# ctlab/metacherchant

Hardware: AMD Instinct MI355X
Metric: k-mers/s processed (count+BFS) at k=31 (higher is better)
Workload: dtype int64

## Files before the change

metacherchant_amd/csrc/count_pipeline.h:

```cpp
#pragma once
#include <utility>
#include "kmer_device.h"

namespace mc {

constexpr int PT_THREADS = 1024;
constexpr int PT_ITEMS = 8;
constexpr int PT_TILE = PT_THREADS * PT_ITEMS;
constexpr int PT_MAX_BUCKETS = 512;
constexpr int PT_MAX_BUCKETS_KEYS = 1024;
constexpr int PT_MAX_LEAVES2 = 1024;
constexpr int PT_MAX_BUCKETS1_SK = 2048;
constexpr int SK_LEAVES_LG = 21;
constexpr int P3_THREADS = 512;
constexpr uint32_t REGION_SLOTS = 1u << MC_REGION_LG;
constexpr uint32_t CURSOR1_STRIDE = 32;
constexpr int PT_SEGMENTS = 256;

__host__ __device__ __forceinline__ uint32_t mulhi32(uint32_t bin, uint32_t n) { return (uint32_t)(((uint64_t)bin * n) >> 32); }

struct ScatterLds {
    uint64_t key[PT_TILE];
    uint32_t hint[PT_TILE];
    uint32_t rel[PT_TILE];
// ... 437 lines not shown

#ifndef MC_P1W_MIN_WAVES
#define MC_P1W_MIN_WAVES 4
#endif
#ifndef MC_P1W_PREFETCH_WORDS
#define MC_P1W_PREFETCH_WORDS 1
#endif
#ifndef MC_P1W_COMPACT
#define MC_P1W_COMPACT 1
#endif
#ifndef MC_P1W_THREADS
#define MC_P1W_THREADS 1024
#endif
constexpr int P1W_THREADS = MC_P1W_THREADS;
constexpr int P1W_WAVES = P1W_THREADS / 64;
constexpr uint32_t P1W_TILE = 62 * PT_ITEMS;
constexpr int P1W_SEGMENTS = 1024;
static_assert(PT_MAX_LEAVES2 <= PT_THREADS && PT_MAX_BUCKETS_KEYS <= PT_THREADS, "one thread per leaf cursor");
static_assert(P1W_SEGMENTS <= PT_THREADS && P1W_SEGMENTS >= PT_SEGMENTS, "k_sk2_scatter scans one segment count per thread");

__device__ __forceinline__ uint32_t wave_incl_sum(uint32_t v)
{
    v += (uint32_t)__builtin_amdgcn_update_dpp(0, (int)v, 0x111, 0xF, 0xF, true);
    v += (uint32_t)__builtin_amdgcn_update_dpp(0, (int)v, 0x112, 0xF, 0xF, true);
    v += (uint32_t)__builtin_amdgcn_update_dpp(0, (int)v, 0x114, 0xF, 0xF, true);
    v += (uint32_t)__builtin_amdgcn_update_dpp(0, (int)v, 0x118, 0xF, 0xF, true);
    v += (uint32_t)__builtin_amdgcn_update_dpp(0, (int)v, 0x142, 0xA, 0xF, false);
    v += (uint32_t)__builtin_amdgcn_update_dpp(0, (int)v, 0x143, 0xC, 0xF, false);
    return v;
}

// ... 15 lines not shown
__device__ __forceinline__ uint32_t sk_start_bits(uint32_t lane, uint32_t valid, uint32_t brk)
{
    static_assert(N <= 16 && N <= (int)MAXW && (MAXW & (MAXW - 1)) == 0 && MAXW <= 32, "one deep start a lane at most");
    const unsigned long long holders = __ballot(brk != 0);
    const unsigned long long below = holders & ((1ull << lane) - 1ull);
    const uint32_t P = below ? 63u - (uint32_t)__builtin_clzll(below) : 0u;
    const uint32_t bp = (uint32_t)__shfl((int)brk, (int)P);
    const uint32_t cur = P * N + (31u - (uint32_t)__builtin_clz(bp | 1u));
    const uint32_t low = (brk & (0u - brk)) - 1u;
    const uint32_t deep = (1u << ((cur - lane * N) & (MAXW - 1u))) & low;
    return valid & (brk | deep);
}

__device__ __forceinline__ uint32_t p1w_wave(uint32_t tid) { return (uint32_t)__builtin_amdgcn_readfirstlane((int)(tid >> 6)); }

struct alignas(16) Sk1wLds {
    uint32_t wcur[PT_MAX_BUCKETS1_SK];
    uint32_t starts[P1W_WAVES][24];
    uint32_t brk[P1W_WAVES][20];
#if MC_P1W_COMPACT
    uint64_t wst[P1W_WAVES][24];
    uint32_t hst[P1W_WAVES][64 * PT_ITEMS];
    uint16_t squeue[P1W_WAVES][64 * PT_ITEMS];
#endif
};

__device__ __forceinline__ uint32_t wave_from_next(uint32_t x)
{
    return (uint32_t)__builtin_amdgcn_update_dpp(0, (int)x, 0x130, 0xF, 0xF, true);
}
__device__ __forceinline__ uint32_t wave_from_prev(uint32_t x, uint32_t first)
{
    return (uint32_t)__builtin_amdgcn_update_dpp((int)first, (int)x, 0x138, 0xF, 0xF, false);
}

__device__ __forceinline__ uint64_t p1w_bits(uint64_t W0, uint64_t W1, uint64_t W2, uint32_t q)
{
    const bool up = q >= 32;
    const uint64_t a = up ? W1 : W0, b = up ? W2 : W1;
    const uint32_t sh = 2 * (q & 31);
    return (a << sh) | ((b >> 1) >> (63 - sh));
}

constexpr uint32_t SKC_REL_BITS = 22;
constexpr uint32_t SKB_MAX_CELLS = 16384;
template <bool ON> struct Sk1wFine { uint32_t h[ON ? SKB_MAX_CELLS : 1]; uint32_t win[ON ? PT_MAX_BUCKETS : 1]; };
struct SkBinned { uint32_t sub, fine; uint32_t *fine_rows; unsigned long long *owner_windows; };
template <bool OWNERS, bool COMPACT = false, bool BINNED = false>
__global__ void __launch_bounds__(P1W_THREADS, MC_P1W_MIN_WAVES) k_sk1w_extract(
    const uint64_t *__restrict__ words, const uint64_t *__restrict__ offsets, uint64_t n_reads, uint64_t base_lo,
    uint64_t n_bases, uint64_t n_tiles, const uint32_t *__restrict__ first_read, int k, uint32_t np1, uint32_t *seg_counts,
    uint64_t cap, uint4 *out_recs, uint32_t *out_ptrs, SkSpill sp, uint64_t ptr_base, uint32_t chunk_tiles = 0, uint32_t m2 = 0,
    SkBinned bn = SkBinned{1, 1, nullptr, nullptr})
{
    static_assert(!(OWNERS && COMPACT), "the compact form is for the single-GPU pipeline");
    static_assert(!BINNED || OWNERS, "fine buckets are the owners' business");
    __shared__ Sk1wLds L;
    __shared__ Sk1wFine<BINNED> F;
    const uint32_t tid = threadIdx.x, lane = tid & 63u, wv = p1w_wave(tid);
    for (uint32_t i = tid; i < PT_MAX_BUCKETS1_SK; i += P1W_THREADS) L.wcur[i] = 0;
    if (BINNED) {
        for (uint32_t i = tid; i < np1 * bn.fine; i += P1W_THREADS) F.h[i] = 0;
        for (uint32_t i = tid; i < np1; i += P1W_THREADS) F.win[i] = 0;
    }
    auto bucket_of = [&](uint32_t hsel, uint32_t bin, uint32_t n_win) -> uint32_t {
        if (BINNED) {
            const uint32_t o = sk_owner(hsel, np1);
            atomicAdd(&F.h[o * bn.fine + mulhi32(bin, bn.fine)], 1u);
            atomicAdd(&F.win[o], n_win);
            return o * bn.sub + mulhi32(bin, bn.sub);
        }
        return OWNERS ? sk_owner(hsel, np1) : mulhi32(bin, np1);
    };
    uint32_t *starts = L.starts[wv];
    uint32_t *brkw = L.brk[wv];
    uint8_t *brkb = reinterpret_cast<uint8_t *>(brkw);
#if MC_P1W_COMPACT
    uint64_t *wst = L.wst[wv];
    uint32_t *hst = L.hst[wv];
    uint16_t *squeue = L.squeue[wv];
    if (lane < 24) wst[lane] = 0;
#endif
    if (lane < 20) brkw[lane] = lane == 0 ? 0u : 0xFFFFFFFFu;
    __syncthreads();
    const int w = k - SK_M + 1;
    const uint64_t last_word = (n_bases + 31) / 32;
    const uint64_t seg_base = (uint64_t)blockIdx.x * cap, bucket_stride = (uint64_t)gridDim.x * cap;
    const uint64_t wave_id = (uint64_t)blockIdx.x * P1W_WAVES + wv, n_waves = (uint64_t)gridDim.x * P1W_WAVES;

    uint64_t pfW0 = 0, pfW1 = 0, pfW2 = 0, pf_off = ~0ull;
    uint32_t pf_first = 0;
    auto load_words = [&](uint64_t tile) {
        const int64_t p0 = (int64_t)(tile * P1W_TILE) + (int64_t)lane * PT_ITEMS;
        const int64_t wi0 = (p0 - 7) >> 5;
        pfW0 = wi0 >= 0 ? words[min((uint64_t)wi0, last_word)] : 0ull;
        pfW1 = words[min((uint64_t)(wi0 + 1), last_word)];
        pfW2 = words[min((uint64_t)(wi0 + 2), last_word)];
    };
    auto prefetch = [&](uint64_t tile) {
        if (tile >= n_tiles) return;
        if (MC_P1W_PREFETCH_WORDS) load_words(tile);
        pf_first = first_read[tile];
        const uint64_t r = (uint64_t)pf_first + lane;
        pf_off = r < n_reads ? offsets[r] : ~0ull;
    };
    const uint64_t chunk_lo = base_lo / P1W_TILE + (uint64_t)blockIdx.x * chunk_tiles;
    const uint64_t tile_end = COMPACT ? min(n_tiles, chunk_lo + chunk_tiles) : n_tiles;
    const uint64_t tile0 = COMPACT ? chunk_lo + wv : base_lo / P1W_TILE + wave_id;
    const uint64_t tile_step = COMPACT ? (uint64_t)P1W_WAVES : n_waves;
    prefetch(tile0);
    for (uint64_t tile = tile0; tile < tile_end; tile += tile_step) {
        const uint64_t lo = tile * (uint64_t)P1W_TILE;
        const int64_t bm_lo = (int64_t)lo - 64;
        const uint64_t bm_hi = lo + 640;
        if (!MC_P1W_PREFETCH_WORDS) load_words(tile);
        const uint64_t W0 = pfW0, W1 = pfW1, W2 = pfW2;
        uint64_t s = pf_off;
        const uint32_t my_first = pf_first;
        prefetch(tile + tile_step);
        const uint64_t p0 = lo + (uint64_t)lane * PT_ITEMS;
        const uint32_t off0 = (uint32_t)((int64_t)p0 - 32 * (((int64_t)p0 - 7) >> 5));

        if (lane < 24) starts[lane] = 0;
        __builtin_amdgcn_fence(__ATOMIC_RELEASE, "wavefront");
        __builtin_amdgcn_wave_barrier();
        for (uint64_t r = (uint64_t)my_first + lane;; r += 64) {
            const bool in = r < n_reads && s < bm_hi;
            if (in) {
                const int64_t rel = (int64_t)s - bm_lo;
                if (rel >= 0) atomicOr(&starts[(uint32_t)rel >> 5], 1u << ((uint32_t)rel & 31));
            }
            if (__ballot(!in)) break;
            s = r + 64 < n_reads ? offsets[r + 64] : ~0ull;
        }
        __builtin_amdgcn_fence(__ATOMIC_RELEASE, "wavefront");
        __builtin_amdgcn_wave_barrier();
        uint32_t ws[4];
        {
            const uint32_t bit0 = lane * 8 + 56, wd = bit0 >> 5, sh = bit0 & 31;
            const uint32_t d0 = starts[wd], d1 = starts[wd + 1], d2 = starts[wd + 2], d3 = starts[wd + 3], d4 = starts[wd + 4];
            ws[0] = __builtin_amdgcn_alignbit(d1, d0, sh);
            ws[1] = __builtin_amdgcn_alignbit(d2, d1, sh);
            ws[2] = __builtin_amdgcn_alignbit(d3, d2, sh);
            ws[3] = __builtin_amdgcn_alignbit(d4, d3, sh);
        }

        uint32_t hh[24];
        {
            const uint64_t A = p1w_bits(W0, W1, W2, off0);
            uint32_t f = (uint32_t)(A >> (64 - 2 * SK_M)), r = sk_rc_mmer(f);
            hh[0] = sk_order(f < r ? f : r);
#pragma unroll
            for (int i = 1; i < 8; i++) {
                const uint32_t nb = (uint32_t)(A >> (62 - 2 * (i + SK_M - 1))) & 3u;
                f = ((f << 2) | nb) & SK_MMASK;
                r = (r >> 2) | ((3u - nb) << (2 * (SK_M - 1)));
                hh[i] = sk_order(f < r ? f : r);
            }
#pragma unroll
            for (int i = 0; i < 8; i++) hh[8 + i] = wave_from_next(hh[i]);
#pragma unroll
            for (int i = 0; i < 8; i++) hh[16 + i] = wave_from_next(hh[8 + i]);
        }
        uint32_t hmin[PT_ITEMS];
#define SK_CASE(W)                                                                             \
    case W: {                                                                                  \
        uint32_t core = hh[7];                                                                 \
        _Pragma("unroll") for (int i = 8; i < W; i++) core = min(core, hh[i]);                 \
        uint32_t suf = SK_NONE;                                                                \
        hmin[7] = core;                                                                        \
        _Pragma("unroll") for (int j = 6; j >= 0; j--) { suf = min(suf, hh[j]); hmin[j] = min(suf, core); } \
        uint32_t pre = SK_NONE;                                                                \
        _Pragma("unroll") for (int j = 1; j < PT_ITEMS; j++) { pre = min(pre, hh[W + j - 1]); hmin[j] = min(hmin[j], pre); } \
    } break;
        switch (w) {
            SK_CASE(9) SK_CASE(10) SK_CASE(11) SK_CASE(12) SK_CASE(13) SK_CASE(14) SK_CASE(15) SK_CASE(16)
        default:
            SK_CASE(17)
        }
#undef SK_CASE

        uint32_t valid_bits;
        {
            uint64_t S = ((((uint64_t)ws[1]) << 32) | ws[0]) >> 9;
            uint32_t width = 1;
            for (; 2 * width <= (uint32_t)k - 1; width *= 2) S |= S >> width;
            S |= S >> ((uint32_t)k - 1 - width);
            uint32_t edge = lane < 62 ? 0xFFu : 0u;
            if (lo < base_lo || lo + P1W_TILE + (uint64_t)k > n_bases + 1) {
                edge = 0;
                if (lane < 62 && p0 + (uint64_t)k <= n_bases) {
                    const uint64_t jmax = n_bases - (uint64_t)k - p0;
                    const uint32_t jm = jmax < 7 ? (uint32_t)jmax : 7u;
                    const uint32_t j0 = p0 >= base_lo ? 0u : (base_lo - p0 < 8 ? (uint32_t)(base_lo - p0) : 8u);
                    edge = ((2u << jm) - 1u) & ~((1u << j0) - 1u) & 0xFFu;
                }
            }
            valid_bits = ~(uint32_t)S & edge;
        }
        const uint32_t last = (valid_bits >> (PT_ITEMS - 1)) & 1u ? hmin[PT_ITEMS - 1] : SK_NONE;
        const uint32_t prev = wave_from_prev(last, SK_NONE);
        const uint32_t brk_bits = sk_break_bits<PT_ITEMS, false>(hmin, valid_bits, prev);
        brkb[2 + lane] = (uint8_t)brk_bits;
        __builtin_amdgcn_fence(__ATOMIC_RELEASE, "wavefront");
        __builtin_amdgcn_wave_barrier();
        const uint32_t start_bits = sk_start_bits<PT_ITEMS, SK_MAX_WINDOWS>(lane, valid_bits, brk_bits);

#if MC_P1W_COMPACT
        {
            const uint32_t cnt = (uint32_t)__builtin_popcount(start_bits);
            const uint32_t incl = wave_incl_sum(cnt);
            const uint32_t total = (uint32_t)__builtin_amdgcn_readlane((int)incl, 63);
            uint32_t at = incl - cnt;
            for (uint32_t todo = start_bits; todo; todo &= todo - 1) squeue[at++] = (uint16_t)(lane * PT_ITEMS + (uint32_t)__builtin_ctz(todo));
            const uint32_t r7 = (uint32_t)(((int64_t)lo - 7) & 31);
            const uint32_t idx0 = (r7 + lane * PT_ITEMS) >> 5;
            wst[idx0] = W0; wst[idx0 + 1] = W1; wst[idx0 + 2] = W2;
            *reinterpret_cast<uint4 *>(&hst[lane * PT_ITEMS]) = make_uint4(hmin[0], hmin[1], hmin[2], hmin[3]);
            *reinterpret_cast<uint4 *>(&hst[lane * PT_ITEMS + 4]) = make_uint4(hmin[4], hmin[5], hmin[6], hmin[7]);
            __builtin_amdgcn_fence(__ATOMIC_RELEASE, "wavefront");
            __builtin_amdgcn_wave_barrier();
            for (uint32_t i = lane; i < total; i += 64) {
                const uint32_t wi = squeue[i];
                const uint32_t b0 = 17u + wi;
                const uint32_t ahead = __builtin_amdgcn_alignbit(brkw[(b0 >> 5) + 1], brkw[b0 >> 5], b0 & 31u) & 0x7FFFu;
                const uint32_t n = ahead ? (uint32_t)__builtin_ctz(ahead) + 1u : SK_MAX_WINDOWS;
                const uint32_t len = n + (uint32_t)k - 1;
                const uint32_t q = wi + 7u + r7, wq = q >> 5, sh = 2u * (q & 31u);
                const uint64_t A = wst[wq], B = wst[wq + 1], C = wst[wq + 2];
                const uint64_t X0 = (A << sh) | ((B >> 1) >> (63u - sh)), X1 = (B << sh) | ((C >> 1) >> (63u - sh));
                uint64_t hi = X0 >> 4;
                uint32_t tail = (uint32_t)(((X0 & 0xFull) << 28) | (X1 >> 36));
                if (len <= 30) { hi &= ~0ull << (60 - 2 * len); tail = 0; }
                else tail &= len >= 46 ? ~0u : ~0u << (2 * (46 - len));
// ... 29 lines not shown
        }
        for (uint32_t todo = start_bits; todo; todo &= todo - 1) {
            const uint32_t j = (uint32_t)__builtin_ctz(todo);
            const uint32_t ahead = (uint32_t)(bw >> (17 + j)) & 0x7FFFu;
            const uint32_t n = ahead ? (uint32_t)__builtin_ctz(ahead) + 1u : SK_MAX_WINDOWS;
            const uint32_t len = n + (uint32_t)k - 1;
            const uint32_t q = off0 + j;
            const uint64_t X0 = p1w_bits(W0, W1, W2, q), X1 = p1w_bits(W1, W2, 0ull, q);
            uint64_t hi = X0 >> 4;
            uint32_t tail = (uint32_t)(((X0 & 0xFull) << 28) | (X1 >> 36));
            if (len <= 30) { hi &= ~0ull << (60 - 2 * len); tail = 0; }
            else tail &= len >= 46 ? ~0u : ~0u << (2 * (46 - len));
            hi |= (uint64_t)(n - 1) << 60;
            uint32_t hsel = hmin[0];
#pragma unroll
            for (int qq = 1; qq < PT_ITEMS; qq++) hsel = j == (uint32_t)qq ? hmin[qq] : hsel;
            const uint32_t bin = sk_bin(hsel);
            const uint32_t d = bucket_of(hsel, bin, n);
            uint4 rec;
            rec.x = bin; rec.y = tail; rec.z = (uint32_t)hi; rec.w = (uint32_t)(hi >> 32);
            const uint64_t dst = atomicAdd(&L.wcur[d], 1u);
            if (dst < cap) {
                const uint64_t at = seg_base + (uint64_t)d * bucket_stride + dst;
                if (COMPACT) {
                    const uint32_t rel = (uint32_t)(tile - chunk_lo) * P1W_TILE + lane * PT_ITEMS + j;
                    rec.x = rel | ((mulhi32(bin, np1 * m2) - d * m2) << SKC_REL_BITS);
                    out_recs[at] = rec;
                } else {
                    out_recs[at] = rec;
                    out_ptrs[at] = ptr_base == ~0ull ? 0u : ptr_encode(ptr_base + p0 + j);
                }
            } else {
                sk_spill_push(sp, rec);
            }
        }
#endif
    }
    __syncthreads();
    const uint32_t n_buckets = BINNED ? np1 * bn.sub : np1;
    for (uint32_t d = tid; d < n_buckets; d += P1W_THREADS)
// ... 1588 lines not shown
```

metacherchant_amd/csrc/mcgpu.hip:

```cpp
#include <unistd.h>

#include <cmath>
#include <cstdlib>
#include <cstring>
#include <thread>

#include "context.h"
#include "count_pipeline.h"
#include "count_long.h"

TablePool g_table_pool;
ScratchPool g_scratch_pool;
thread_local std::string g_create_err;


__global__ void k_fill_empty(Slot *slots, uint64_t n)
{
    const uint64_t stride = (uint64_t)gridDim.x * blockDim.x;
    for (uint64_t i = (uint64_t)blockIdx.x * blockDim.x + threadIdx.x; i < n; i += stride) {
        uint4 v;
        v.x = 0xFFFFFFFFu; v.y = 0xFFFFFFFFu; v.z = 0; v.w = 0;
        *reinterpret_cast<uint4 *>(slots + i) = v;
    }
}
// ... 1058 lines not shown
    }
    uint64_t n_leaves, np1;
    uint32_t g;
    if (const char *why = plan_levels(c, n_records != 0, &n_leaves, &g, &np1)) return fail(c, MC_EINVAL, "internal: %s (%llu table regions)", why, (unsigned long long)c->n_regions);
    pl->b1 = (uint32_t)np1;
    pl->b2 = (uint32_t)(n_leaves / np1);
    pl->g = g;
    pl->wb = wb;
    pl->np1 = np1;
    pl->n_leaves = n_leaves;
    pl->sk = n_records != 0;
    if (pl->b2 <= 1) pl->pieces = pieces = 1;
    if (!level2_only) {
        const uint64_t chunk = (compact_tiles + nseg1 - 1) / std::max<uint32_t>(nseg1, 1);
        pl->compact = compact_tiles && c->sw.sk_compact && pl->sk && pl->b2 > 1 && pl->b2 <= (1u << (32 - SKC_REL_BITS)) && g == 0 &&
                      chunk * P1W_TILE <= (1ull << SKC_REL_BITS) && !(pl->guessed && c->virgin);
        pl->vleaf = false;
        if (!pl->compact && !lng && c->sw.sk_vleaf && !c->no_vleaf && compact_tiles && c->sw.sk_compact && pl->sk && g == 0 && chunk * P1W_TILE <= (1ull << SKC_REL_BITS) &&
            pl->guessed && c->virgin && c->mm_k > 0 && np1 == PT_MAX_BUCKETS && c->n_regions <= (uint64_t)PT_MAX_BUCKETS * 1024) {
            uint64_t r2 = 2 * PT_MAX_BUCKETS;
            while (r2 < c->n_regions) r2 *= 2;
            if (r2 != c->n_regions) {
                table_release(c, c->slots, c->slots_bytes);
                c->slots = nullptr;
                int rc = table_alloc(c, r2);
                if (rc) return rc;
                n_leaves = r2;
                pl->b2 = (uint32_t)(n_leaves / np1);
                pl->n_leaves = n_leaves;
            }
            pl->compact = pl->vleaf = true;
        }
        if (lng) pl->compact = compact_tiles && pl->sk && pl->b2 > 1 && pl->b2 <= 1024 && g == 0 && chunk * P1L_TILE < (1ull << 32) &&
// ... 198 lines not shown
    const bool virgin0 = c->virgin;
    auto launch_p2 = [&] {
        static bool told = false;
        if (c->sw.ingest_debug && !told) {
            told = true;
            fprintf(stderr, "[count] level-1 stream %p (%llu records a segment), level-2 stream %p (%llu a leaf), table %p\n", (void *)P.a_recs,
                    (unsigned long long)pl.cap1, (void *)P.b_recs, (unsigned long long)pl.cap2, (void *)c->slots);
        }
        if (pl.lng)
            hipLaunchKernelGGL((k_sk2_scatter_compact<2, 2>), dim3((unsigned)np1), dim3(PT_THREADS), 0, c->stream, P.a_recs, pl.cap1,
                               P.seg_counts1, (uint32_t)np1, pl.b2, P.cursors2, pl.cap2, P.b_recs, pl.sks, pl.nseg1, c->cur_ptr_base, pl.pos0,
                               (uint64_t)pl.chunk_tiles * P1L_TILE);
        else if (pl.sk && pl.compact && !pl.listed)
            hipLaunchKernelGGL(k_sk2_scatter_compact<MC_SK2C_ITEMS>, dim3((unsigned)np1), dim3(PT_THREADS), 0, c->stream, P.a_recs, pl.cap1,
                               P.seg_counts1, (uint32_t)np1, pl.b2, P.cursors2, pl.cap2, P.b_recs, pl.sks, pl.nseg1, c->cur_ptr_base, pl.pos0,
                               (uint64_t)pl.chunk_tiles * P1W_TILE, pl.vleaf ? 10u - (uint32_t)__builtin_ctz(pl.b2) : 0u);
        else if (pl.listed)
            hipLaunchKernelGGL((k_sk2_scatter_staged<MC_SK2_ITEMS, true, false>), dim3((unsigned)np1), dim3(PT_THREADS), 0, c->stream, pl.in_recs, pl.in_ptrs, (uint64_t)0,
                               P.seg_counts1, (uint32_t)np1, pl.b1, pl.b2, P.cursors2, pl.cap2, P.b_recs, nullptr, pl.sks, pl.nseg1, P.skb_seg_start, nullptr);
        else if (pl.sk)
            hipLaunchKernelGGL(k_sk2_scatter_staged<MC_SK2_ITEMS>, dim3((unsigned)np1), dim3(PT_THREADS), 0, c->stream, P.a_recs, P.a_hints, pl.cap1,
                               P.seg_counts1, (uint32_t)np1, pl.b1, pl.b2, P.cursors2, pl.cap2, P.b_recs, P.b_hints, pl.sks, pl.nseg1);
        else
            hipLaunchKernelGGL(k_p2_scatter, dim3((unsigned)np1), dim3(PT_THREADS), 0, c->stream, P.a_keys, P.a_hints, pl.cap1,
                               P.seg_counts1, (uint32_t)np1, pl.b1, pl.b2, P.cursors2, pl.cap2, P.b_keys, P.b_hints, pl.sp, c->mm_k);
    };
    auto resize_for_batch = [&](uint64_t sample_leaves) -> int {
        std::vector<uint32_t> st(sample_leaves), nw(sample_leaves);
        HIPCHK(c, hipMemcpy(st.data(), P.leaf_state, sample_leaves * sizeof(uint32_t), hipMemcpyDeviceToHost));
        HIPCHK(c, hipMemcpy(nw.data(), P.leaf_new, sample_leaves * sizeof(uint32_t), hipMemcpyDeviceToHost));
        uint64_t merged = 0, added = 0;
// ... 320 lines not shown
static int add_reads_partitioned_once(mc_ctx *c, const uint64_t *d_words, const uint64_t *d_off, uint64_t r0, uint64_t r1,
                                      uint64_t base0, uint64_t end_abs, uint64_t wb)
{
    mc_ctx::Pipe &P = c->pipe;
    PipePlan pl;
    const uint64_t nr = r1 - r0;
    if (hash_bins(c)) {
        int lrc = add_reads_long(c, d_words, d_off, r0, r1, base0, end_abs, wb);
        if (lrc == 1) return count_batch_direct(c, d_words, d_off, r0, r1, base0, end_abs, wb);
        if (lrc != 4) return lrc;
        lrc = to_hash_regions(c, 3);
        if (lrc) return lrc;
        if (end_abs - base0 > max_run_bases(c, (double)wb / (double)std::max<uint64_t>(end_abs - base0, 1))) return RC_RESPLIT;
    }
    const uint64_t n_records = c->mm_k ? sk_records_bound(c, wb, nr) : 0;
    int rc = pipe_prepare(c, wb, &pl, n_records, n_records ? (uint32_t)P1W_SEGMENTS : (uint32_t)PT_SEGMENTS,
                          n_records || wb < (3ull << 29) ? 1u : (uint32_t)std::min<uint64_t>(8, (wb + (1ull << 30) - 1) >> 30), false,
                          n_records ? (end_abs + P1W_TILE - 1) / P1W_TILE - base0 / P1W_TILE : 0);
    if (rc) return rc;
    const uint32_t pieces = pl.pieces;
    const uint64_t *offs = d_off + r0;
    const uint32_t tile_size = pl.sk ? P1W_TILE : (uint32_t)PT_TILE;
    const uint64_t n_tiles_abs = (end_abs + tile_size - 1) / tile_size;
    rc = ensure_buf(c, &P.tile_first, &P.tiles1_cap, n_tiles_abs);
    if (rc) return rc;
    double ms1 = 0;
    if (pieces > 1) {
        const uint64_t t_first = base0 / tile_size, per = (n_tiles_abs - t_first + pieces - 1) / pieces;
        for (uint32_t i = 0; i < 2 * pieces; i++)
            if (!c->ev_seq[i]) HIPCHK(c, hipEventCreate(&c->ev_seq[i]));
        HIPCHK(c, hipEventRecord(c->ev0, c->stream));
        launch_tile_first(c, offs, nr, n_tiles_abs, P.tile_first, tile_size);
        for (uint32_t pc = 0; pc < pieces; pc++) {
            const uint64_t lo_t = t_first + pc * per, hi_t = std::min<uint64_t>(n_tiles_abs, lo_t + per);
            if (lo_t < hi_t)
                launch_p1_reads(c, d_words, offs, nr, pc == 0 ? base0 : lo_t * tile_size, end_abs, hi_t, P.tile_first, pl.b1, P.seg_counts1, pl.cap1,
                                P.a_keys, P.a_hints, pl.sp, 0, nullptr);
// ... 6 lines not shown
        HIPCHK(c, hipGetLastError());
        HIPCHK(c, hipEventSynchronize(c->ev_seq[2 * pieces - 1]));
        double ms2 = 0;
        for (uint32_t pc = 0; pc < pieces; pc++) {
            float f1 = 0, f2 = 0;
            HIPCHK(c, hipEventElapsedTime(&f1, pc ? c->ev_seq[2 * pc - 1] : c->ev0, c->ev_seq[2 * pc]));
            HIPCHK(c, hipEventElapsedTime(&f2, c->ev_seq[2 * pc], c->ev_seq[2 * pc + 1]));
            ms1 += f1;
            ms2 += f2;
        }
        rc = pipe_finish(c, pl, ms1, true, ms2, false, true);
    } else {
        HIPCHK(c, hipEventRecord(c->ev_t[0], c->stream));
        launch_tile_first(c, offs, nr, n_tiles_abs, P.tile_first, tile_size);
        if (pl.sk && pl.compact) {
            pl.pos0 = base0 / P1W_TILE * P1W_TILE;
            if (c->sw.ingest_debug)
                fprintf(stderr, "[count] compact records: %u buckets x %u leaves%s, %u tiles a segment from base %llu\n", pl.b1, pl.vleaf ? 1024u : pl.b2,
                        pl.vleaf ? " (whatever the table: it is sized behind the first level)" : "", pl.chunk_tiles, (unsigned long long)pl.pos0);
            hipLaunchKernelGGL((k_sk1w_extract<false, true>), dim3(P1W_SEGMENTS), dim3(P1W_THREADS), 0, c->stream, d_words, offs, nr, base0, end_abs,
                               n_tiles_abs, P.tile_first, c->cfg.k, pl.b1, P.seg_counts1, pl.cap1, P.a_recs, nullptr, pl.sks, c->cur_ptr_base,
                               pl.chunk_tiles, pl.vleaf ? 1024u : pl.b2);
        }
        else if (pl.sk)
            hipLaunchKernelGGL(k_sk1w_extract<false>, dim3(P1W_SEGMENTS), dim3(P1W_THREADS), 0, c->stream, d_words, offs, nr, base0, end_abs,
                               n_tiles_abs, P.tile_first, c->cfg.k, pl.b1, P.seg_counts1, pl.cap1, P.a_recs, P.a_hints, pl.sks, c->cur_ptr_base);
        else
            launch_p1_reads(c, d_words, offs, nr, base0, end_abs, n_tiles_abs, P.tile_first, pl.b1, P.seg_counts1, pl.cap1, P.a_keys,
                            P.a_hints, pl.sp, 0, nullptr);
        HIPCHK(c, hipGetLastError());
        rc = pipe_resize_by_sample(c, pl, n_records);
// ... 974 lines not shown
    HIPCHK(c, hipMemcpyAsync(&first_off, d_off, 8, hipMemcpyDeviceToHost, c->stream));
    HIPCHK(c, hipMemcpyAsync(&last_off, d_off + n_reads, 8, hipMemcpyDeviceToHost, c->stream));
    HIPCHK(c, hipStreamSynchronize(c->stream));
    if (last_off != n_bases)
        return fail(c, MC_EINVAL, "mc_extract_superkmers_dev: read_offsets[n_reads]=%llu but n_bases=%llu",
                    (unsigned long long)last_off, (unsigned long long)n_bases);
    {
        const int64_t in_store = c->extract_in_store;
        c->extract_in_store = -1;
        int rrc = rs_append(c, d_words, first_off, last_off, in_store);
        if (rrc) return rrc;
    }
    c->solid_list_fresh = false;
    const uint64_t bound = sk_records_bound(c, n_bases - first_off, n_reads);
    const uint32_t nseg = P1W_SEGMENTS;
    uint64_t seg_cap = (uint64_t)((double)bound / (double)n_owners / (double)nseg * 1.25) + 64;
    {
        const uint64_t n_waves = (uint64_t)nseg * P1W_WAVES;
        const uint64_t tiles = (last_off - first_off + P1W_TILE - 1) / P1W_TILE + 1, per_wg = (tiles + n_waves - 1) / n_waves * P1W_WAVES;
        const double per_tile = (double)bound / (double)std::max<uint64_t>(tiles - 1, 1);
        seg_cap = std::max<uint64_t>(seg_cap, (uint64_t)((double)per_wg * per_tile / (double)n_owners * 1.3) + 64);
    }
    if ((uint64_t)n_owners * nseg * seg_cap >= 0xFFFFFFFFull)
        return fail(c, MC_EINVAL, "mc_extract_superkmers_dev: batch too large (split the reads)");
    const uint64_t n_tiles_abs = (last_off + P1W_TILE - 1) / P1W_TILE;
    int rc = ensure_buf(c, &P.tile_first, &P.tiles1_cap, n_tiles_abs);
    if (!rc) rc = ensure_buf(c, &P.a_recs, &P.a_recs_cap, (uint64_t)n_owners * nseg * seg_cap);
    if (!rc) rc = ensure_buf(c, &P.a_hints, &P.a_hints_cap, (uint64_t)n_owners * nseg * seg_cap);
    if (!rc) rc = ensure_buf(c, &P.seg_counts1, &P.segs1_cap, (uint64_t)n_owners * nseg);
    if (rc) return rc;
    if (!P.flags) {
        HIPCHK(c, hipMalloc(reinterpret_cast<void **>(&P.flags), 4 * sizeof(uint32_t) + sizeof(unsigned long long)));
        P.spill_count = reinterpret_cast<unsigned long long *>(P.flags + 4);
    }
    HIPCHK(c, hipMemsetAsync(P.flags, 0, 4 * sizeof(uint32_t) + sizeof(unsigned long long), c->stream));
    DevBuf<unsigned long long> d_piece, d_owner;
    HIPCHK(c, d_piece.alloc((uint64_t)n_owners * nseg));
    HIPCHK(c, d_owner.alloc(n_owners + 1));
    const SkSpill none{nullptr, P.spill_count, 0, P.flags};
    launch_tile_first(c, d_off, n_reads, n_tiles_abs, P.tile_first, P1W_TILE);
    hipLaunchKernelGGL(k_sk1w_extract<true>, dim3(nseg), dim3(P1W_THREADS), 0, c->stream, d_words, d_off, n_reads, first_off,
                       last_off, n_tiles_abs, P.tile_first, c->cfg.k, n_owners, P.seg_counts1, seg_cap, P.a_recs, P.a_hints, none, c->cur_ptr_base);
    hipLaunchKernelGGL(k_sk_pack_offsets, dim3(1), dim3(1024), 0, c->stream, P.seg_counts1, n_owners, d_piece.p, d_owner.p, nseg);
    hipLaunchKernelGGL(k_sk_pack, dim3(std::min<uint32_t>(n_owners * nseg, 4096)), dim3(256), 0, c->stream, P.a_recs, P.a_hints,
                       P.seg_counts1, seg_cap, d_piece.p, n_owners * nseg, reinterpret_cast<uint4 *>(d_recs), d_bins, cap);
    HIPCHK(c, hipGetLastError());
    std::vector<unsigned long long> h_owner(n_owners + 1);
    uint32_t lost = 0;
    HIPCHK(c, hipMemcpyAsync(h_owner.data(), d_owner.p, (n_owners + 1) * sizeof(unsigned long long), hipMemcpyDeviceToHost, c->stream));
    HIPCHK(c, hipMemcpyAsync(&lost, P.flags, sizeof lost, hipMemcpyDeviceToHost, c->stream));
    HIPCHK(c, hipStreamSynchronize(c->stream));
    if (lost) return fail(c, MC_EOVERFLOW, "mc_extract_superkmers_dev: more super-k-mers than expected (unusually short runs); use mc_extract_keys_dev");
    if (h_owner[n_owners] > cap)
        return fail(c, MC_EINVAL, "mc_extract_superkmers_dev: %llu records but capacity %llu", h_owner[n_owners], (unsigned long long)cap);
    for (uint32_t o = 0; o <= n_owners; o++) owner_offsets[o] = h_owner[o];
// ... 45 lines not shown
    HIPCHK(c, hipMemcpyAsync(&first_off, d_off, 8, hipMemcpyDeviceToHost, c->stream));
    HIPCHK(c, hipMemcpyAsync(&last_off, d_off + n_reads, 8, hipMemcpyDeviceToHost, c->stream));
    HIPCHK(c, hipStreamSynchronize(c->stream));
    if (last_off != n_bases)
        return fail(c, MC_EINVAL, "mc_extract_superkmers_binned_dev: read_offsets[n_reads]=%llu but n_bases=%llu",
                    (unsigned long long)last_off, (unsigned long long)n_bases);
    {
        const int64_t in_store = c->extract_in_store;
        c->extract_in_store = -1;
        int rrc = rs_append(c, d_words, first_off, last_off, in_store);
        if (rrc) return rrc;
    }
    c->solid_list_fresh = false;
    const uint64_t bound = sk_records_bound(c, n_bases - first_off, n_reads);
    const uint32_t nseg = P1W_SEGMENTS, n_buckets = n_owners * sub;
    uint64_t seg_cap = (uint64_t)((double)bound / (double)n_buckets / (double)nseg * 1.25) + 64;
    {
        const uint64_t n_waves = (uint64_t)nseg * P1W_WAVES;
        const uint64_t tiles = (last_off - first_off + P1W_TILE - 1) / P1W_TILE + 1, per_wg = (tiles + n_waves - 1) / n_waves * P1W_WAVES;
        const double per_tile = (double)bound / (double)std::max<uint64_t>(tiles - 1, 1);
        seg_cap = std::max<uint64_t>(seg_cap, (uint64_t)((double)per_wg * per_tile / (double)n_buckets * 1.3) + 64);
    }
    if ((uint64_t)n_buckets * nseg * seg_cap >= 0xFFFFFFFFull)
        return fail(c, MC_EINVAL, "mc_extract_superkmers_binned_dev: batch too large (split the reads)");
    const uint64_t n_tiles_abs = (last_off + P1W_TILE - 1) / P1W_TILE;
    int rc = ensure_buf(c, &P.tile_first, &P.tiles1_cap, n_tiles_abs);
    if (!rc) rc = ensure_buf(c, &P.a_recs, &P.a_recs_cap, (uint64_t)n_buckets * nseg * seg_cap);
    if (!rc) rc = ensure_buf(c, &P.a_hints, &P.a_hints_cap, (uint64_t)n_buckets * nseg * seg_cap);
    if (!rc) rc = ensure_buf(c, &P.seg_counts1, &P.segs1_cap, (uint64_t)n_buckets * nseg);
    if (!rc) rc = ensure_buf(c, &P.skb_rows, &P.skb_rows_cap, (uint64_t)nseg * n_cells);
    if (!rc) rc = ensure_buf(c, &P.skb_cell_start, &P.skb_cell_start_cap, n_cells);
    if (!rc) rc = ensure_buf(c, &P.skb_small, &P.skb_small_cap, (uint64_t)P1W_SEGMENTS + 2 * PT_MAX_BUCKETS + 8);
    if (rc) return rc;
    if (!P.flags) {
        HIPCHK(c, hipMalloc(reinterpret_cast<void **>(&P.flags), 4 * sizeof(uint32_t) + sizeof(unsigned long long)));
        P.spill_count = reinterpret_cast<unsigned long long *>(P.flags + 4);
    }
    HIPCHK(c, hipMemsetAsync(P.flags, 0, 4 * sizeof(uint32_t) + sizeof(unsigned long long), c->stream));
    unsigned long long *d_owner = P.skb_small, *d_win = P.skb_small + n_owners + 1;
    HIPCHK(c, hipMemsetAsync(d_win, 0, n_owners * sizeof(unsigned long long), c->stream));
    const SkSpill none{nullptr, P.spill_count, 0, P.flags};
    launch_tile_first(c, d_off, n_reads, n_tiles_abs, P.tile_first, P1W_TILE);
    hipLaunchKernelGGL((k_sk1w_extract<true, false, true>), dim3(nseg), dim3(P1W_THREADS), 0, c->stream, d_words, d_off, n_reads, first_off,
                       last_off, n_tiles_abs, P.tile_first, c->cfg.k, n_owners, P.seg_counts1, seg_cap, P.a_recs, P.a_hints, none, c->cur_ptr_base,
                       0u, 0u, SkBinned{sub, n_fine, P.skb_rows, d_win});
    hipLaunchKernelGGL(k_skb_colsum, dim3((unsigned)((n_cells + 255) / 256), 16), dim3(256), 0, c->stream, P.skb_rows, nseg, (uint32_t)n_cells, d_fine_counts);
    hipLaunchKernelGGL(k_skb_offsets, dim3(1), dim3(1024), 0, c->stream, d_fine_counts, n_owners, n_fine, P.skb_cell_start, d_owner);
    hipLaunchKernelGGL((k_sk2_scatter_staged<MC_SK2_ITEMS, false, true>), dim3(n_buckets), dim3(PT_THREADS), 0, c->stream, P.a_recs, P.a_hints, seg_cap,
                       P.seg_counts1, n_buckets, sub, n_fine / sub, nullptr, cap, reinterpret_cast<uint4 *>(d_recs), d_ptrs, none, nseg, nullptr, P.skb_cell_start);
    HIPCHK(c, hipGetLastError());
    std::vector<unsigned long long> h(2 * n_owners + 1);
    uint32_t lost = 0;
    HIPCHK(c, hipMemcpyAsync(h.data(), d_owner, (2 * n_owners + 1) * sizeof(unsigned long long), hipMemcpyDeviceToHost, c->stream));
    HIPCHK(c, hipMemcpyAsync(&lost, P.flags, sizeof lost, hipMemcpyDeviceToHost, c->stream));
    HIPCHK(c, hipStreamSynchronize(c->stream));
    if (lost) return fail(c, MC_EOVERFLOW, "mc_extract_superkmers_binned_dev: more super-k-mers than expected (unusually short runs); use mc_extract_keys_dev");
    if (h[n_owners] > cap)
// ... 557 lines not shown
```

Measured before the change: 65.14 billion.

## Process sixteen positions per lane in single-GPU super-k-mer extraction

New measurement: 67.12 billion, median of 6. +3.0%, better.

```diff
diff --git a/metacherchant_amd/csrc/count_pipeline.h b/metacherchant_amd/csrc/count_pipeline.h
--- a/metacherchant_amd/csrc/count_pipeline.h
+++ b/metacherchant_amd/csrc/count_pipeline.h
@@ -475,7 +475,8 @@
 #endif
 constexpr int P1W_THREADS = MC_P1W_THREADS;
 constexpr int P1W_WAVES = P1W_THREADS / 64;
-constexpr uint32_t P1W_TILE = 62 * PT_ITEMS;
+constexpr int p1w_items(bool owners) { return owners || !MC_P1W_COMPACT ? PT_ITEMS : 16; }
+constexpr uint32_t p1w_tile(bool owners) { return 62u * (uint32_t)p1w_items(owners); }
 constexpr int P1W_SEGMENTS = 1024;
 static_assert(PT_MAX_LEAVES2 <= PT_THREADS && PT_MAX_BUCKETS_KEYS <= PT_THREADS, "one thread per leaf cursor");
 static_assert(P1W_SEGMENTS <= PT_THREADS && P1W_SEGMENTS >= PT_SEGMENTS, "k_sk2_scatter scans one segment count per thread");
@@ -521,16 +522,63 @@
 
 __device__ __forceinline__ uint32_t p1w_wave(uint32_t tid) { return (uint32_t)__builtin_amdgcn_readfirstlane((int)(tid >> 6)); }
 
-struct alignas(16) Sk1wLds {
+template <int NI> struct alignas(16) Sk1wLds {
+    static constexpr int AUX = 2 * NI + 4;
     uint32_t wcur[PT_MAX_BUCKETS1_SK];
-    uint32_t starts[P1W_WAVES][24];
-    uint32_t brk[P1W_WAVES][20];
+    uint32_t starts[P1W_WAVES][AUX];
+    uint32_t brk[P1W_WAVES][AUX];
 #if MC_P1W_COMPACT
-    uint64_t wst[P1W_WAVES][24];
-    uint32_t hst[P1W_WAVES][64 * PT_ITEMS];
-    uint16_t squeue[P1W_WAVES][64 * PT_ITEMS];
+    uint64_t wst[P1W_WAVES][AUX];
+    uint32_t hst[P1W_WAVES][64 * NI];
+    uint16_t squeue[P1W_WAVES][64 * NI];
 #endif
 };
+
+template <int W, int B, int N>
+__device__ __forceinline__ void sk_core_minima8(const uint32_t (&hh)[32], uint32_t (&hmin)[N])
+{
+    static_assert(W >= 9 && W <= 17 && B + 8 <= N && B + W + 6 < 32, "windows of 9 .. 17 hashes");
+    uint32_t core = hh[B + 7];
+#pragma unroll
+    for (int i = 8; i < W; i++) core = min(core, hh[B + i]);
+    uint32_t suf = SK_NONE;
+    hmin[B + 7] = core;
+#pragma unroll
+    for (int j = 6; j >= 0; j--) { suf = min(suf, hh[B + j]); hmin[B + j] = min(suf, core); }
+    uint32_t pre = SK_NONE;
+#pragma unroll
+    for (int j = 1; j < 8; j++) { pre = min(pre, hh[B + W + j - 1]); hmin[B + j] = min(hmin[B + j], pre); }
+}
+
+template <int W>
+__device__ __forceinline__ void sk_block_minima16(const uint32_t (&hh)[32], uint32_t (&hmin)[16])
+{
+    static_assert(W >= 15 && W <= 17, "no window begins behind the first of block 1");
+    constexpr int A = W < 16 ? W : 16;
+    constexpr int NP1 = W == 15 ? W : A - 1;
+    uint32_t s0[W], p1[W];
+    s0[W - 1] = hh[W - 1];
+#pragma unroll
+    for (int i = W - 2; i >= 0; i--) s0[i] = min(s0[i + 1], hh[i]);
+    p1[0] = hh[W];
+#pragma unroll
+    for (int i = 1; i < NP1; i++) p1[i] = min(p1[i - 1], hh[W + i]);
+    hmin[0] = s0[0];
+#pragma unroll
+    for (int j = 1; j < A; j++) hmin[j] = min(s0[j], p1[j - 1]);
+    if constexpr (W == 15) hmin[W] = p1[W - 1];
+}
+
+template <int W, int N>
+__device__ __forceinline__ void sk_window_minima(const uint32_t (&hh)[32], uint32_t (&hmin)[N])
+{
+    static_assert(N == 8 || N == 16, "8 or 16 positions a lane");
+    if constexpr (N == 16 && W >= 15) sk_block_minima16<W>(hh, hmin);
+    else {
+        sk_core_minima8<W, 0>(hh, hmin);
+        if constexpr (N == 16) sk_core_minima8<W, 8>(hh, hmin);
+    }
+}
 
 __device__ __forceinline__ uint32_t wave_from_next(uint32_t x)
 {
@@ -553,7 +601,7 @@
 constexpr uint32_t SKB_MAX_CELLS = 16384;
 template <bool ON> struct Sk1wFine { uint32_t h[ON ? SKB_MAX_CELLS : 1]; uint32_t win[ON ? PT_MAX_BUCKETS : 1]; };
 struct SkBinned { uint32_t sub, fine; uint32_t *fine_rows; unsigned long long *owner_windows; };
-template <bool OWNERS, bool COMPACT = false, bool BINNED = false>
+template <bool OWNERS, bool COMPACT = false, bool BINNED = false, int NI = p1w_items(OWNERS)>
 __global__ void __launch_bounds__(P1W_THREADS, MC_P1W_MIN_WAVES) k_sk1w_extract(
     const uint64_t *__restrict__ words, const uint64_t *__restrict__ offsets, uint64_t n_reads, uint64_t base_lo,
     uint64_t n_bases, uint64_t n_tiles, const uint32_t *__restrict__ first_read, int k, uint32_t np1, uint32_t *seg_counts,
@@ -562,7 +610,10 @@
 {
     static_assert(!(OWNERS && COMPACT), "the compact form is for the single-GPU pipeline");
     static_assert(!BINNED || OWNERS, "fine buckets are the owners' business");
-    __shared__ Sk1wLds L;
+    static_assert(NI == 8 || (NI == 16 && MC_P1W_COMPACT), "8 or 16 positions a lane");
+    constexpr uint32_t P1W_TILE = 62u * NI;
+    constexpr uint32_t AUX = Sk1wLds<NI>::AUX;
+    __shared__ Sk1wLds<NI> L;
     __shared__ Sk1wFine<BINNED> F;
     const uint32_t tid = threadIdx.x, lane = tid & 63u, wv = p1w_wave(tid);
     for (uint32_t i = tid; i < PT_MAX_BUCKETS1_SK; i += P1W_THREADS) L.wcur[i] = 0;
@@ -581,14 +632,13 @@
     };
     uint32_t *starts = L.starts[wv];
     uint32_t *brkw = L.brk[wv];
-    uint8_t *brkb = reinterpret_cast<uint8_t *>(brkw);
 #if MC_P1W_COMPACT
     uint64_t *wst = L.wst[wv];
     uint32_t *hst = L.hst[wv];
     uint16_t *squeue = L.squeue[wv];
-    if (lane < 24) wst[lane] = 0;
-#endif
-    if (lane < 20) brkw[lane] = lane == 0 ? 0u : 0xFFFFFFFFu;
+    if (lane < AUX) wst[lane] = 0;
+#endif
+    if (lane < AUX) brkw[lane] = lane == 0 ? 0u : 0xFFFFFFFFu;
     __syncthreads();
     const int w = k - SK_M + 1;
     const uint64_t last_word = (n_bases + 31) / 32;
@@ -598,7 +648,7 @@
     uint64_t pfW0 = 0, pfW1 = 0, pfW2 = 0, pf_off = ~0ull;
     uint32_t pf_first = 0;
     auto load_words = [&](uint64_t tile) {
-        const int64_t p0 = (int64_t)(tile * P1W_TILE) + (int64_t)lane * PT_ITEMS;
+        const int64_t p0 = (int64_t)(tile * P1W_TILE) + (int64_t)lane * NI;
         const int64_t wi0 = (p0 - 7) >> 5;
         pfW0 = wi0 >= 0 ? words[min((uint64_t)wi0, last_word)] : 0ull;
         pfW1 = words[min((uint64_t)(wi0 + 1), last_word)];
@@ -619,16 +669,16 @@
     for (uint64_t tile = tile0; tile < tile_end; tile += tile_step) {
         const uint64_t lo = tile * (uint64_t)P1W_TILE;
         const int64_t bm_lo = (int64_t)lo - 64;
-        const uint64_t bm_hi = lo + 640;
+        const uint64_t bm_hi = (uint64_t)(bm_lo + 32 * (int64_t)AUX);
         if (!MC_P1W_PREFETCH_WORDS) load_words(tile);
         const uint64_t W0 = pfW0, W1 = pfW1, W2 = pfW2;
         uint64_t s = pf_off;
         const uint32_t my_first = pf_first;
         prefetch(tile + tile_step);
-        const uint64_t p0 = lo + (uint64_t)lane * PT_ITEMS;
+        const uint64_t p0 = lo + (uint64_t)lane * NI;
         const uint32_t off0 = (uint32_t)((int64_t)p0 - 32 * (((int64_t)p0 - 7) >> 5));
 
-        if (lane < 24) starts[lane] = 0;
+        if (lane < AUX) starts[lane] = 0;
         __builtin_amdgcn_fence(__ATOMIC_RELEASE, "wavefront");
         __builtin_amdgcn_wave_barrier();
         for (uint64_t r = (uint64_t)my_first + lane;; r += 64) {
@@ -642,50 +692,45 @@
         }
         __builtin_amdgcn_fence(__ATOMIC_RELEASE, "wavefront");
         __builtin_amdgcn_wave_barrier();
-        uint32_t ws[4];
+        uint32_t ws[2];
         {
-            const uint32_t bit0 = lane * 8 + 56, wd = bit0 >> 5, sh = bit0 & 31;
-            const uint32_t d0 = starts[wd], d1 = starts[wd + 1], d2 = starts[wd + 2], d3 = starts[wd + 3], d4 = starts[wd + 4];
+            const uint32_t bit0 = lane * NI + 56, wd = bit0 >> 5, sh = bit0 & 31;
+            const uint32_t d0 = starts[wd], d1 = starts[wd + 1], d2 = starts[wd + 2];
             ws[0] = __builtin_amdgcn_alignbit(d1, d0, sh);
             ws[1] = __builtin_amdgcn_alignbit(d2, d1, sh);
-            ws[2] = __builtin_amdgcn_alignbit(d3, d2, sh);
-            ws[3] = __builtin_amdgcn_alignbit(d4, d3, sh);
-        }
-
-        uint32_t hh[24];
+        }
+
+        uint32_t hh[32];
         {
             const uint64_t A = p1w_bits(W0, W1, W2, off0);
             uint32_t f = (uint32_t)(A >> (64 - 2 * SK_M)), r = sk_rc_mmer(f);
             hh[0] = sk_order(f < r ? f : r);
 #pragma unroll
-            for (int i = 1; i < 8; i++) {
+            for (int i = 1; i < NI; i++) {
                 const uint32_t nb = (uint32_t)(A >> (62 - 2 * (i + SK_M - 1))) & 3u;
                 f = ((f << 2) | nb) & SK_MMASK;
                 r = (r >> 2) | ((3u - nb) << (2 * (SK_M - 1)));
                 hh[i] = sk_order(f < r ? f : r);
             }
 #pragma unroll
-            for (int i = 0; i < 8; i++) hh[8 + i] = wave_from_next(hh[i]);
-#pragma unroll
-            for (int i = 0; i < 8; i++) hh[16 + i] = wave_from_next(hh[8 + i]);
-        }
-        uint32_t hmin[PT_ITEMS];
-#define SK_CASE(W)                                                                             \
-    case W: {                                                                                  \
-        uint32_t core = hh[7];                                                                 \
-        _Pragma("unroll") for (int i = 8; i < W; i++) core = min(core, hh[i]);                 \
-        uint32_t suf = SK_NONE;                                                                \
-        hmin[7] = core;                                                                        \
-        _Pragma("unroll") for (int j = 6; j >= 0; j--) { suf = min(suf, hh[j]); hmin[j] = min(suf, core); } \
-        uint32_t pre = SK_NONE;                                                                \
-        _Pragma("unroll") for (int j = 1; j < PT_ITEMS; j++) { pre = min(pre, hh[W + j - 1]); hmin[j] = min(hmin[j], pre); } \
-    } break;
+            for (int i = 0; i < NI; i++) hh[NI + i] = wave_from_next(hh[i]);
+            if constexpr (NI == 8) {
+#pragma unroll
+                for (int i = 0; i < 8; i++) hh[16 + i] = wave_from_next(hh[8 + i]);
+            }
+        }
+        uint32_t hmin[NI];
         switch (w) {
-            SK_CASE(9) SK_CASE(10) SK_CASE(11) SK_CASE(12) SK_CASE(13) SK_CASE(14) SK_CASE(15) SK_CASE(16)
-        default:
-            SK_CASE(17)
-        }
-#undef SK_CASE
+        case 9: sk_window_minima<9>(hh, hmin); break;
+        case 10: sk_window_minima<10>(hh, hmin); break;
+        case 11: sk_window_minima<11>(hh, hmin); break;
+        case 12: sk_window_minima<12>(hh, hmin); break;
+        case 13: sk_window_minima<13>(hh, hmin); break;
+        case 14: sk_window_minima<14>(hh, hmin); break;
+        case 15: sk_window_minima<15>(hh, hmin); break;
+        case 16: sk_window_minima<16>(hh, hmin); break;
+        default: sk_window_minima<17>(hh, hmin); break;
+        }
 
         uint32_t valid_bits;
         {
@@ -693,25 +738,27 @@
             uint32_t width = 1;
             for (; 2 * width <= (uint32_t)k - 1; width *= 2) S |= S >> width;
             S |= S >> ((uint32_t)k - 1 - width);
-            uint32_t edge = lane < 62 ? 0xFFu : 0u;
+            constexpr uint32_t ALL = (1u << NI) - 1u;
+            uint32_t edge = lane < 62 ? ALL : 0u;
             if (lo < base_lo || lo + P1W_TILE + (uint64_t)k > n_bases + 1) {
                 edge = 0;
                 if (lane < 62 && p0 + (uint64_t)k <= n_bases) {
                     const uint64_t jmax = n_bases - (uint64_t)k - p0;
-                    const uint32_t jm = jmax < 7 ? (uint32_t)jmax : 7u;
-                    const uint32_t j0 = p0 >= base_lo ? 0u : (base_lo - p0 < 8 ? (uint32_t)(base_lo - p0) : 8u);
-                    edge = ((2u << jm) - 1u) & ~((1u << j0) - 1u) & 0xFFu;
+                    const uint32_t jm = jmax < (uint64_t)(NI - 1) ? (uint32_t)jmax : (uint32_t)(NI - 1);
+                    const uint32_t j0 = p0 >= base_lo ? 0u : (base_lo - p0 < (uint64_t)NI ? (uint32_t)(base_lo - p0) : (uint32_t)NI);
+                    edge = ((2u << jm) - 1u) & ~((1u << j0) - 1u) & ALL;
                 }
             }
             valid_bits = ~(uint32_t)S & edge;
         }
-        const uint32_t last = (valid_bits >> (PT_ITEMS - 1)) & 1u ? hmin[PT_ITEMS - 1] : SK_NONE;
+        const uint32_t last = (valid_bits >> (NI - 1)) & 1u ? hmin[NI - 1] : SK_NONE;
         const uint32_t prev = wave_from_prev(last, SK_NONE);
-        const uint32_t brk_bits = sk_break_bits<PT_ITEMS, false>(hmin, valid_bits, prev);
-        brkb[2 + lane] = (uint8_t)brk_bits;
+        const uint32_t brk_bits = sk_break_bits<NI, false>(hmin, valid_bits, prev);
+        if constexpr (NI == 8) reinterpret_cast<uint8_t *>(brkw)[2 + lane] = (uint8_t)brk_bits;
+        else reinterpret_cast<uint16_t *>(brkw)[1 + lane] = (uint16_t)brk_bits;
         __builtin_amdgcn_fence(__ATOMIC_RELEASE, "wavefront");
         __builtin_amdgcn_wave_barrier();
-        const uint32_t start_bits = sk_start_bits<PT_ITEMS, SK_MAX_WINDOWS>(lane, valid_bits, brk_bits);
+        const uint32_t start_bits = sk_start_bits<NI, SK_MAX_WINDOWS>(lane, valid_bits, brk_bits);
 
 #if MC_P1W_COMPACT
         {
@@ -719,12 +766,12 @@
             const uint32_t incl = wave_incl_sum(cnt);
             const uint32_t total = (uint32_t)__builtin_amdgcn_readlane((int)incl, 63);
             uint32_t at = incl - cnt;
-            for (uint32_t todo = start_bits; todo; todo &= todo - 1) squeue[at++] = (uint16_t)(lane * PT_ITEMS + (uint32_t)__builtin_ctz(todo));
+            for (uint32_t todo = start_bits; todo; todo &= todo - 1) squeue[at++] = (uint16_t)(lane * NI + (uint32_t)__builtin_ctz(todo));
             const uint32_t r7 = (uint32_t)(((int64_t)lo - 7) & 31);
-            const uint32_t idx0 = (r7 + lane * PT_ITEMS) >> 5;
+            const uint32_t idx0 = (r7 + lane * NI) >> 5;
             wst[idx0] = W0; wst[idx0 + 1] = W1; wst[idx0 + 2] = W2;
-            *reinterpret_cast<uint4 *>(&hst[lane * PT_ITEMS]) = make_uint4(hmin[0], hmin[1], hmin[2], hmin[3]);
-            *reinterpret_cast<uint4 *>(&hst[lane * PT_ITEMS + 4]) = make_uint4(hmin[4], hmin[5], hmin[6], hmin[7]);
+#pragma unroll
+            for (int j = 0; j < NI; j += 4) *reinterpret_cast<uint4 *>(&hst[lane * NI + j]) = make_uint4(hmin[j], hmin[j + 1], hmin[j + 2], hmin[j + 3]);
             __builtin_amdgcn_fence(__ATOMIC_RELEASE, "wavefront");
             __builtin_amdgcn_wave_barrier();
             for (uint32_t i = lane; i < total; i += 64) {
@@ -784,7 +831,7 @@
             hi |= (uint64_t)(n - 1) << 60;
             uint32_t hsel = hmin[0];
 #pragma unroll
-            for (int qq = 1; qq < PT_ITEMS; qq++) hsel = j == (uint32_t)qq ? hmin[qq] : hsel;
+            for (int qq = 1; qq < NI; qq++) hsel = j == (uint32_t)qq ? hmin[qq] : hsel;
             const uint32_t bin = sk_bin(hsel);
             const uint32_t d = bucket_of(hsel, bin, n);
             uint4 rec;
@@ -793,7 +840,7 @@
             if (dst < cap) {
                 const uint64_t at = seg_base + (uint64_t)d * bucket_stride + dst;
                 if (COMPACT) {
-                    const uint32_t rel = (uint32_t)(tile - chunk_lo) * P1W_TILE + lane * PT_ITEMS + j;
+                    const uint32_t rel = (uint32_t)(tile - chunk_lo) * P1W_TILE + lane * NI + j;
                     rec.x = rel | ((mulhi32(bin, np1 * m2) - d * m2) << SKC_REL_BITS);
                     out_recs[at] = rec;
                 } else {
diff --git a/metacherchant_amd/csrc/mcgpu.hip b/metacherchant_amd/csrc/mcgpu.hip
--- a/metacherchant_amd/csrc/mcgpu.hip
+++ b/metacherchant_amd/csrc/mcgpu.hip
@@ -1096,9 +1096,9 @@
     if (!level2_only) {
         const uint64_t chunk = (compact_tiles + nseg1 - 1) / std::max<uint32_t>(nseg1, 1);
         pl->compact = compact_tiles && c->sw.sk_compact && pl->sk && pl->b2 > 1 && pl->b2 <= (1u << (32 - SKC_REL_BITS)) && g == 0 &&
-                      chunk * P1W_TILE <= (1ull << SKC_REL_BITS) && !(pl->guessed && c->virgin);
+                      chunk * p1w_tile(false) <= (1ull << SKC_REL_BITS) && !(pl->guessed && c->virgin);
         pl->vleaf = false;
-        if (!pl->compact && !lng && c->sw.sk_vleaf && !c->no_vleaf && compact_tiles && c->sw.sk_compact && pl->sk && g == 0 && chunk * P1W_TILE <= (1ull << SKC_REL_BITS) &&
+        if (!pl->compact && !lng && c->sw.sk_vleaf && !c->no_vleaf && compact_tiles && c->sw.sk_compact && pl->sk && g == 0 && chunk * p1w_tile(false) <= (1ull << SKC_REL_BITS) &&
             pl->guessed && c->virgin && c->mm_k > 0 && np1 == PT_MAX_BUCKETS && c->n_regions <= (uint64_t)PT_MAX_BUCKETS * 1024) {
             uint64_t r2 = 2 * PT_MAX_BUCKETS;
             while (r2 < c->n_regions) r2 *= 2;
@@ -1327,7 +1327,7 @@
         else if (pl.sk && pl.compact && !pl.listed)
             hipLaunchKernelGGL(k_sk2_scatter_compact<MC_SK2C_ITEMS>, dim3((unsigned)np1), dim3(PT_THREADS), 0, c->stream, P.a_recs, pl.cap1,
                                P.seg_counts1, (uint32_t)np1, pl.b2, P.cursors2, pl.cap2, P.b_recs, pl.sks, pl.nseg1, c->cur_ptr_base, pl.pos0,
-                               (uint64_t)pl.chunk_tiles * P1W_TILE, pl.vleaf ? 10u - (uint32_t)__builtin_ctz(pl.b2) : 0u);
+                               (uint64_t)pl.chunk_tiles * p1w_tile(false), pl.vleaf ? 10u - (uint32_t)__builtin_ctz(pl.b2) : 0u);
         else if (pl.listed)
             hipLaunchKernelGGL((k_sk2_scatter_staged<MC_SK2_ITEMS, true, false>), dim3((unsigned)np1), dim3(PT_THREADS), 0, c->stream, pl.in_recs, pl.in_ptrs, (uint64_t)0,
                                P.seg_counts1, (uint32_t)np1, pl.b1, pl.b2, P.cursors2, pl.cap2, P.b_recs, nullptr, pl.sks, pl.nseg1, P.skb_seg_start, nullptr);
@@ -1678,13 +1678,14 @@
         if (end_abs - base0 > max_run_bases(c, (double)wb / (double)std::max<uint64_t>(end_abs - base0, 1))) return RC_RESPLIT;
     }
     const uint64_t n_records = c->mm_k ? sk_records_bound(c, wb, nr) : 0;
+    constexpr uint32_t sk_tile = p1w_tile(false);
     int rc = pipe_prepare(c, wb, &pl, n_records, n_records ? (uint32_t)P1W_SEGMENTS : (uint32_t)PT_SEGMENTS,
                           n_records || wb < (3ull << 29) ? 1u : (uint32_t)std::min<uint64_t>(8, (wb + (1ull << 30) - 1) >> 30), false,
-                          n_records ? (end_abs + P1W_TILE - 1) / P1W_TILE - base0 / P1W_TILE : 0);
+                          n_records ? (end_abs + sk_tile - 1) / sk_tile - base0 / sk_tile : 0);
     if (rc) return rc;
     const uint32_t pieces = pl.pieces;
     const uint64_t *offs = d_off + r0;
-    const uint32_t tile_size = pl.sk ? P1W_TILE : (uint32_t)PT_TILE;
+    const uint32_t tile_size = pl.sk ? sk_tile : (uint32_t)PT_TILE;
     const uint64_t n_tiles_abs = (end_abs + tile_size - 1) / tile_size;
     rc = ensure_buf(c, &P.tile_first, &P.tiles1_cap, n_tiles_abs);
     if (rc) return rc;
@@ -1721,7 +1722,7 @@
         HIPCHK(c, hipEventRecord(c->ev_t[0], c->stream));
         launch_tile_first(c, offs, nr, n_tiles_abs, P.tile_first, tile_size);
         if (pl.sk && pl.compact) {
-            pl.pos0 = base0 / P1W_TILE * P1W_TILE;
+            pl.pos0 = base0 / sk_tile * sk_tile;
             if (c->sw.ingest_debug)
                 fprintf(stderr, "[count] compact records: %u buckets x %u leaves%s, %u tiles a segment from base %llu\n", pl.b1, pl.vleaf ? 1024u : pl.b2,
                         pl.vleaf ? " (whatever the table: it is sized behind the first level)" : "", pl.chunk_tiles, (unsigned long long)pl.pos0);
@@ -2726,16 +2727,17 @@
     c->solid_list_fresh = false;
     const uint64_t bound = sk_records_bound(c, n_bases - first_off, n_reads);
     const uint32_t nseg = P1W_SEGMENTS;
+    constexpr uint32_t own_tile = p1w_tile(true);
     uint64_t seg_cap = (uint64_t)((double)bound / (double)n_owners / (double)nseg * 1.25) + 64;
     {
         const uint64_t n_waves = (uint64_t)nseg * P1W_WAVES;
-        const uint64_t tiles = (last_off - first_off + P1W_TILE - 1) / P1W_TILE + 1, per_wg = (tiles + n_waves - 1) / n_waves * P1W_WAVES;
+        const uint64_t tiles = (last_off - first_off + own_tile - 1) / own_tile + 1, per_wg = (tiles + n_waves - 1) / n_waves * P1W_WAVES;
         const double per_tile = (double)bound / (double)std::max<uint64_t>(tiles - 1, 1);
         seg_cap = std::max<uint64_t>(seg_cap, (uint64_t)((double)per_wg * per_tile / (double)n_owners * 1.3) + 64);
     }
     if ((uint64_t)n_owners * nseg * seg_cap >= 0xFFFFFFFFull)
         return fail(c, MC_EINVAL, "mc_extract_superkmers_dev: batch too large (split the reads)");
-    const uint64_t n_tiles_abs = (last_off + P1W_TILE - 1) / P1W_TILE;
+    const uint64_t n_tiles_abs = (last_off + own_tile - 1) / own_tile;
     int rc = ensure_buf(c, &P.tile_first, &P.tiles1_cap, n_tiles_abs);
     if (!rc) rc = ensure_buf(c, &P.a_recs, &P.a_recs_cap, (uint64_t)n_owners * nseg * seg_cap);
     if (!rc) rc = ensure_buf(c, &P.a_hints, &P.a_hints_cap, (uint64_t)n_owners * nseg * seg_cap);
@@ -2750,7 +2752,7 @@
     HIPCHK(c, d_piece.alloc((uint64_t)n_owners * nseg));
     HIPCHK(c, d_owner.alloc(n_owners + 1));
     const SkSpill none{nullptr, P.spill_count, 0, P.flags};
-    launch_tile_first(c, d_off, n_reads, n_tiles_abs, P.tile_first, P1W_TILE);
+    launch_tile_first(c, d_off, n_reads, n_tiles_abs, P.tile_first, own_tile);
     hipLaunchKernelGGL(k_sk1w_extract<true>, dim3(nseg), dim3(P1W_THREADS), 0, c->stream, d_words, d_off, n_reads, first_off,
                        last_off, n_tiles_abs, P.tile_first, c->cfg.k, n_owners, P.seg_counts1, seg_cap, P.a_recs, P.a_hints, none, c->cur_ptr_base);
     hipLaunchKernelGGL(k_sk_pack_offsets, dim3(1), dim3(1024), 0, c->stream, P.seg_counts1, n_owners, d_piece.p, d_owner.p, nseg);
@@ -2826,16 +2828,17 @@
     c->solid_list_fresh = false;
     const uint64_t bound = sk_records_bound(c, n_bases - first_off, n_reads);
     const uint32_t nseg = P1W_SEGMENTS, n_buckets = n_owners * sub;
+    constexpr uint32_t own_tile = p1w_tile(true);
     uint64_t seg_cap = (uint64_t)((double)bound / (double)n_buckets / (double)nseg * 1.25) + 64;
     {
         const uint64_t n_waves = (uint64_t)nseg * P1W_WAVES;
-        const uint64_t tiles = (last_off - first_off + P1W_TILE - 1) / P1W_TILE + 1, per_wg = (tiles + n_waves - 1) / n_waves * P1W_WAVES;
+        const uint64_t tiles = (last_off - first_off + own_tile - 1) / own_tile + 1, per_wg = (tiles + n_waves - 1) / n_waves * P1W_WAVES;
         const double per_tile = (double)bound / (double)std::max<uint64_t>(tiles - 1, 1);
         seg_cap = std::max<uint64_t>(seg_cap, (uint64_t)((double)per_wg * per_tile / (double)n_buckets * 1.3) + 64);
     }
     if ((uint64_t)n_buckets * nseg * seg_cap >= 0xFFFFFFFFull)
         return fail(c, MC_EINVAL, "mc_extract_superkmers_binned_dev: batch too large (split the reads)");
-    const uint64_t n_tiles_abs = (last_off + P1W_TILE - 1) / P1W_TILE;
+    const uint64_t n_tiles_abs = (last_off + own_tile - 1) / own_tile;
     int rc = ensure_buf(c, &P.tile_first, &P.tiles1_cap, n_tiles_abs);
     if (!rc) rc = ensure_buf(c, &P.a_recs, &P.a_recs_cap, (uint64_t)n_buckets * nseg * seg_cap);
     if (!rc) rc = ensure_buf(c, &P.a_hints, &P.a_hints_cap, (uint64_t)n_buckets * nseg * seg_cap);
@@ -2852,7 +2855,7 @@
     unsigned long long *d_owner = P.skb_small, *d_win = P.skb_small + n_owners + 1;
     HIPCHK(c, hipMemsetAsync(d_win, 0, n_owners * sizeof(unsigned long long), c->stream));
     const SkSpill none{nullptr, P.spill_count, 0, P.flags};
-    launch_tile_first(c, d_off, n_reads, n_tiles_abs, P.tile_first, P1W_TILE);
+    launch_tile_first(c, d_off, n_reads, n_tiles_abs, P.tile_first, own_tile);
     hipLaunchKernelGGL((k_sk1w_extract<true, false, true>), dim3(nseg), dim3(P1W_THREADS), 0, c->stream, d_words, d_off, n_reads, first_off,
                        last_off, n_tiles_abs, P.tile_first, c->cfg.k, n_owners, P.seg_counts1, seg_cap, P.a_recs, P.a_hints, none, c->cur_ptr_base,
                        0u, 0u, SkBinned{sub, n_fine, P.skb_rows, d_win});
```
